# ziesha-network/bazuka

Hardware: NVIDIA B200
Metric: g1_msm_scalars_per_sec (higher is better)
Workload: dtype u32x12 Montgomery (Fp) / u32x8 (Fr) on the GPU; u64 limbs on the CPU

## Files before the change

### bazuka_b200/csrc/ec.cuh

```cuda
#pragma once
#include "ff.cuh"

#if defined(__CUDACC__)
#define BZK_HD_COLD __host__ __device__ __noinline__
#else
#define BZK_HD_COLD
#endif

namespace bzk {

struct Fp2 {
    Fp c0, c1;
    BZK_HD static Fp2 zero() { return Fp2{Fp::zero(), Fp::zero()}; }
    BZK_HD static Fp2 one() { return Fp2{Fp::one(), Fp::zero()}; }
    BZK_HD bool is_zero() const { return c0.is_zero() && c1.is_zero(); }
    BZK_HD bool operator==(const Fp2 &o) const { return c0 == o.c0 && c1 == o.c1; }
    BZK_HD bool operator!=(const Fp2 &o) const { return !(*this == o); }
    BZK_HD friend Fp2 operator+(const Fp2 &a, const Fp2 &b) { return Fp2{a.c0 + b.c0, a.c1 + b.c1}; }
    BZK_HD friend Fp2 operator-(const Fp2 &a, const Fp2 &b) { return Fp2{a.c0 - b.c0, a.c1 - b.c1}; }
    BZK_HD Fp2 neg() const { return Fp2{c0.neg(), c1.neg()}; }
    BZK_HD Fp2 dbl() const { return Fp2{c0.dbl(), c1.dbl()}; }
    BZK_HD friend Fp2 operator*(const Fp2 &a, const Fp2 &b) {
        Fp t0 = a.c0 * b.c0;
        Fp t1 = a.c1 * b.c1;
        Fp t2 = (a.c0 + a.c1) * (b.c0 + b.c1);
        return Fp2{t0 - t1, t2 - t0 - t1};
    }
    BZK_HD Fp2 sqr() const {
        Fp t = c0 * c1;
        return Fp2{(c0 + c1) * (c0 - c1), t.dbl()};
    }
    BZK_HD Fp2 inv() const {
        Fp n = (c0.sqr() + c1.sqr()).inv();
        return Fp2{c0 * n, (c1 * n).neg()};
    }
};

template <class F>
struct Affine {
    F x, y;
    BZK_HD bool is_inf() const { return x.is_zero() && y.is_zero(); }
    BZK_HD static Affine inf() { return Affine{F::zero(), F::zero()}; }
    BZK_HD Affine neg() const { return Affine{x, y.neg()}; }
};

template <class F>
struct Xyzz {
    F X, Y, ZZ, ZZZ;

    BZK_HD static Xyzz inf() { return Xyzz{F::zero(), F::zero(), F::zero(), F::zero()}; }
    BZK_HD bool is_inf() const { return ZZ.is_zero(); }
    BZK_HD static Xyzz from_affine(const Affine<F> &p) {
        if (p.is_inf()) return inf();
        return Xyzz{p.x, p.y, F::one(), F::one()};
    }
    BZK_HD Xyzz neg() const { return Xyzz{X, Y.neg(), ZZ, ZZZ}; }

    BZK_HD_COLD static Xyzz dbl_affine(const Affine<F> &p) {
        if (p.is_inf() || p.y.is_zero()) return inf();
        F U = p.y.dbl();
        F V = U.sqr();
        F W = U * V;
        F S = p.x * V;
        F M = p.x.sqr();
        M = M.dbl() + M;
        Xyzz r;
        r.X = M.sqr() - S.dbl();
        r.Y = M * (S - r.X) - W * p.y;
        r.ZZ = V;
        r.ZZZ = W;
        return r;
    }
    BZK_HD_COLD Xyzz dbl() const {
        if (is_inf() || Y.is_zero()) return inf();
        F U = Y.dbl();
        F V = U.sqr();
        F W = U * V;
        F S = X * V;
        F M = X.sqr();
        M = M.dbl() + M;
        Xyzz r;
        r.X = M.sqr() - S.dbl();
        r.Y = M * (S - r.X) - W * Y;
        r.ZZ = V * ZZ;
        r.ZZZ = W * ZZZ;
        return r;
    }
    BZK_HD void madd(const Affine<F> &p) {
        if (p.is_inf()) return;
        if (is_inf()) {
            X = p.x; Y = p.y; ZZ = F::one(); ZZZ = F::one();
            return;
        }
        F Pd = p.x * ZZ - X;
        F Rd = p.y * ZZZ - Y;
        if (Pd.is_zero()) {
            if (Rd.is_zero()) *this = dbl_affine(p);
            else *this = inf();
            return;
        }
        F PP = Pd.sqr();
        F PPP = Pd * PP;
        F Q = X * PP;
        F X3 = Rd.sqr() - PPP - Q.dbl();
        Y = Rd * (Q - X3) - Y * PPP;
        X = X3;
        ZZ = ZZ * PP;
        ZZZ = ZZZ * PPP;
    }
    BZK_HD_COLD void add(const Xyzz &o) {
        if (o.is_inf()) return;
        if (is_inf()) { *this = o; return; }
        F U1 = X * o.ZZ;
        F U2 = o.X * ZZ;
        F S1 = Y * o.ZZZ;
        F S2 = o.Y * ZZZ;
        F Pd = U2 - U1;
        F Rd = S2 - S1;
        if (Pd.is_zero()) {
            if (Rd.is_zero()) *this = dbl();
            else *this = inf();
            return;
        }
        F PP = Pd.sqr();
        F PPP = Pd * PP;
        F Q = U1 * PP;
        F X3 = Rd.sqr() - PPP - Q.dbl();
        Y = Rd * (Q - X3) - S1 * PPP;
        X = X3;
        ZZ = ZZ * o.ZZ * PP;
        ZZZ = ZZZ * o.ZZZ * PPP;
    }
    BZK_HD_COLD Affine<F> to_affine() const {
        if (is_inf()) return Affine<F>::inf();
        F i = (ZZ * ZZZ).inv();
        return Affine<F>{X * ZZZ * i, Y * ZZ * i};
    }
};

template <class F>
BZK_HD F pair_denominator(const Affine<F> &a, const Affine<F> &b) {
    if (a.is_inf() || b.is_inf()) return F::one();
    const F dx = b.x - a.x;
    if (!dx.is_zero()) return dx;
    if (a.y == b.y && !a.y.is_zero()) return a.y.dbl();
    return F::one();
}
template <class F>
BZK_HD Affine<F> pair_sum(const Affine<F> &a, const Affine<F> &b, const F &dinv) {
    if (a.is_inf()) return b;
    if (b.is_inf()) return a;
    F lam;
    if (a.x != b.x) {
        lam = (b.y - a.y) * dinv;
    } else {
        if (!(a.y == b.y) || a.y.is_zero()) return Affine<F>::inf();
        const F xx = a.x.sqr();
        lam = (xx.dbl() + xx) * dinv;
    }
    Affine<F> r;
    r.x = lam.sqr() - a.x - b.x;
    r.y = lam * (a.x - r.x) - a.y;
    return r;
}

typedef Affine<Fp> G1Affine;
typedef Affine<Fp2> G2Affine;
typedef Xyzz<Fp> G1Xyzz;
typedef Xyzz<Fp2> G2Xyzz;

template <class F>
BZK_HD Xyzz<F> scalar_mul(const Affine<F> &p, const uint32_t k[8]) {
    Xyzz<F> acc = Xyzz<F>::inf();
    for (int i = 255; i >= 0; i--) {
        acc = acc.dbl();
        if ((k[i >> 5] >> (i & 31)) & 1) acc.madd(p);
    }
    return acc;
}

}
```

### bazuka_b200/csrc/ff.cuh

```cuda
#pragma once
#include <stdint.h>
#include <string.h>

#if defined(__CUDACC__)
#define BZK_HD __host__ __device__ __forceinline__
#define BZK_D __device__ __forceinline__
#else
#define BZK_HD inline
#define BZK_D inline
#endif

#if defined(__CUDACC__)
#define BZK_HD_POW __host__ __device__ __noinline__
#else
#define BZK_HD_POW
#endif

namespace bzk {

struct CC {
    uint32_t c;
};

#if defined(__CUDA_ARCH__)
// ... 98 lines not shown
        return r;
    }
    BZK_HD friend Fe operator+(const Fe &a, const Fe &b) {
#if defined(__CUDA_ARCH__)
        return add_limbs32(a, b);
#else
        return add_host64(a, b);
#endif
    }
    BZK_HD friend Fe operator-(const Fe &a, const Fe &b) {
#if defined(__CUDA_ARCH__)
        return sub_limbs32(a, b);
#else
        return sub_host64(a, b);
#endif
    }
    struct HostConsts {
        uint64_t p[N / 2];
        uint64_t inv64;
    };
    static inline const HostConsts &host_consts() {
        static const HostConsts hc = [] {
            HostConsts c;
            for (int i = 0; i < N / 2; i++) c.p[i] = (uint64_t)P::p(2 * i) | ((uint64_t)P::p(2 * i + 1) << 32);
            uint64_t x = (uint64_t)(0u - P::inv());
            x *= 2 - c.p[0] * x;
            c.inv64 = (uint64_t)0 - x;
            return c;
        }();
        return hc;
    }
    static inline Fe add_host64(const Fe &a, const Fe &b) {
        constexpr int M = N / 2;
        uint64_t A[M], B[M], t[M], s[M];
        memcpy(A, a.l, sizeof A);
        memcpy(B, b.l, sizeof B);
        unsigned __int128 c = 0;
        for (int i = 0; i < M; i++) { c += (unsigned __int128)A[i] + B[i]; t[i] = (uint64_t)c; c >>= 64; }
        uint64_t borrow = 0;
        const uint64_t *Pm = host_consts().p;
        for (int i = 0; i < M; i++) {
            const uint64_t pm = Pm[i];
            const unsigned __int128 d = (unsigned __int128)t[i] - pm - borrow;
            s[i] = (uint64_t)d;
            borrow = (uint64_t)(d >> 64) & 1;
        }
        Fe r;
        memcpy(r.l, borrow ? t : s, sizeof t);
        return r;
    }
    static inline Fe sub_host64(const Fe &a, const Fe &b) {
        constexpr int M = N / 2;
        uint64_t A[M], B[M], t[M];
        memcpy(A, a.l, sizeof A);
        memcpy(B, b.l, sizeof B);
        uint64_t borrow = 0;
        for (int i = 0; i < M; i++) {
            const unsigned __int128 d = (unsigned __int128)A[i] - B[i] - borrow;
            t[i] = (uint64_t)d;
            borrow = (uint64_t)(d >> 64) & 1;
        }
        if (borrow) {
            unsigned __int128 c = 0;
            const uint64_t *Pm = host_consts().p;
            for (int i = 0; i < M; i++) {
                const uint64_t pm = Pm[i];
                c += (unsigned __int128)t[i] + pm;
                t[i] = (uint64_t)c;
                c >>= 64;
            }
        }
        Fe r;
        memcpy(r.l, t, sizeof t);
        return r;
    }
    BZK_HD static Fe add_limbs32(const Fe &a, const Fe &b) {
        Fe t;
        CC cc{0};
        t.l[0] = add_cc(a.l[0], b.l[0], cc);
#pragma unroll
        for (int i = 1; i < N; i++) t.l[i] = addc_cc(a.l[i], b.l[i], cc);
        return reduce_once(t);
    }
    BZK_HD static Fe sub_limbs32(const Fe &a, const Fe &b) {
        Fe t;
        CC cc{0};
        t.l[0] = sub_cc(a.l[0], b.l[0], cc);
#pragma unroll
        for (int i = 1; i < N; i++) t.l[i] = subc_cc(a.l[i], b.l[i], cc);
        uint32_t borrow = subc(0, 0, cc);
        CC c2{0};
        t.l[0] = add_cc(t.l[0], borrow & P::p(0), c2);
#pragma unroll
        for (int i = 1; i < N; i++) t.l[i] = addc_cc(t.l[i], borrow & P::p(i), c2);
        return t;
    }
    BZK_HD Fe neg() const { return zero() - *this; }
    BZK_HD Fe dbl() const { return *this + *this; }

    BZK_HD friend Fe operator*(const Fe &a, const Fe &b) {
#if defined(__CUDA_ARCH__) && defined(BZK_MUL_NOINLINE)
        return mul_call(a, b);
#elif defined(__CUDA_ARCH__)
        return mul_evenodd(a, b);
#else
        return mul_host64(a, b);
#endif
    }
#if defined(__CUDACC__)
    __device__ __noinline__ static Fe mul_call(Fe a, Fe b) { return mul_evenodd(a, b); }
#endif
    static inline Fe mul_host64(const Fe &a, const Fe &b) {
        constexpr int M = N / 2;
        uint64_t A[M], B[M], t[M + 2];
        memcpy(A, a.l, sizeof A);
        memcpy(B, b.l, sizeof B);
        const HostConsts &hc = host_consts();
        const uint64_t *Pm = hc.p;
        const uint64_t inv64 = hc.inv64;
        for (int i = 0; i < M + 2; i++) t[i] = 0;
        for (int i = 0; i < M; i++) {
            unsigned __int128 cur;
            uint64_t carry = 0;
            for (int j = 0; j < M; j++) {
                cur = (unsigned __int128)A[j] * B[i] + t[j] + carry;
                t[j] = (uint64_t)cur;
                carry = (uint64_t)(cur >> 64);
            }
            cur = (unsigned __int128)t[M] + carry;
            t[M] = (uint64_t)cur;
            t[M + 1] = (uint64_t)(cur >> 64);
            const uint64_t m = t[0] * inv64;
            cur = (unsigned __int128)m * Pm[0] + t[0];
            carry = (uint64_t)(cur >> 64);
            for (int j = 1; j < M; j++) {
                cur = (unsigned __int128)m * Pm[j] + t[j] + carry;
                t[j - 1] = (uint64_t)cur;
                carry = (uint64_t)(cur >> 64);
            }
            cur = (unsigned __int128)t[M] + carry;
            t[M - 1] = (uint64_t)cur;
            t[M] = t[M + 1] + (uint64_t)(cur >> 64);
        }
        uint64_t s[M], borrow = 0;
        for (int i = 0; i < M; i++) {
            const unsigned __int128 d = (unsigned __int128)t[i] - Pm[i] - borrow;
            s[i] = (uint64_t)d;
            borrow = (uint64_t)(d >> 64) & 1;
        }
        Fe r;
        memcpy(r.l, borrow ? t : s, M * sizeof(uint64_t));
        return r;
    }
    BZK_HD static Fe mul_evenodd(const Fe &a, const Fe &b) {
        uint32_t E[2 * N + 2], O[2 * N + 2];
#pragma unroll
        for (int i = 0; i < 2 * N + 2; i++) E[i] = O[i] = 0;
        CC cc{0};
#pragma unroll
        for (int i = 0; i < N; i++) {
            uint32_t *Pp = (i & 1) ? O : E;
            uint32_t *Q = (i & 1) ? E : O;
            const uint32_t bi = b.l[i];
            if (i == 0) {
#pragma unroll
                for (int j = 0; j < N; j += 2) {
                    Pp[j] = mul_lo(a.l[j], bi);
                    Pp[j + 1] = mul_hi(a.l[j], bi);
                    Q[j + 1] = mul_lo(a.l[j + 1], bi);
                    Q[j + 2] = mul_hi(a.l[j + 1], bi);
                }
            } else {
                Pp[i] = add_cc(Pp[i], Q[i], cc);
#pragma unroll
                for (int j = 1; j < N; j += 2) mad_pair_next(Q[i + j], Q[i + j + 1], a.l[j], bi, cc);
                Q[i + N + 1] = addc(0, 0, cc);
                mad_pair_first(Pp[i], Pp[i + 1], a.l[0], bi, cc);
#pragma unroll
                for (int j = 2; j < N; j += 2) mad_pair_next(Pp[i + j], Pp[i + j + 1], a.l[j], bi, cc);
                Pp[i + N] = addc(Pp[i + N], 0, cc);
            }
            const uint32_t m = mul_lo(Pp[i], P::inv());
            mad_pair_first(Pp[i], Pp[i + 1], m, P::p(0), cc);
#pragma unroll
            for (int j = 2; j < N; j += 2) mad_pair_next(Pp[i + j], Pp[i + j + 1], m, P::p(j), cc);
            Pp[i + N] = addc(Pp[i + N], 0, cc);
            mad_pair_first(Q[i + 1], Q[i + 2], m, P::p(1), cc);
#pragma unroll
            for (int j = 3; j < N; j += 2) mad_pair_next(Q[i + j], Q[i + j + 1], m, P::p(j), cc);
            Q[i + N + 1] = addc(Q[i + N + 1], 0, cc);
        }
        Fe r;
        r.l[0] = add_cc(E[N], O[N], cc);
#pragma unroll
        for (int k = 1; k < N; k++) r.l[k] = addc_cc(E[N + k], O[N + k], cc);
        return reduce_once(r);
    }
    BZK_HD Fe sqr() const { return (*this) * (*this); }

    BZK_HD static void mul_wide(uint32_t out[2 * N], const Fe &a, const Fe &b) {
        uint32_t E[2 * N + 2], O[2 * N + 2];
#pragma unroll
        for (int i = 0; i < 2 * N + 2; i++) E[i] = O[i] = 0;
        CC cc{0};
#pragma unroll
        for (int i = 0; i < N; i++) {
            uint32_t *Pp = (i & 1) ? O : E;
            uint32_t *Q = (i & 1) ? E : O;
            const uint32_t bi = b.l[i];
            if (i == 0) {
#pragma unroll
                for (int j = 0; j < N; j += 2) {
                    Pp[j] = mul_lo(a.l[j], bi);
                    Pp[j + 1] = mul_hi(a.l[j], bi);
                    Q[j + 1] = mul_lo(a.l[j + 1], bi);
                    Q[j + 2] = mul_hi(a.l[j + 1], bi);
                }
            } else {
                mad_pair_first(Q[i + 1], Q[i + 2], a.l[1], bi, cc);
#pragma unroll
                for (int j = 3; j < N; j += 2) mad_pair_next(Q[i + j], Q[i + j + 1], a.l[j], bi, cc);
                Q[i + N + 1] = addc(0, 0, cc);
                mad_pair_first(Pp[i], Pp[i + 1], a.l[0], bi, cc);
#pragma unroll
                for (int j = 2; j < N; j += 2) mad_pair_next(Pp[i + j], Pp[i + j + 1], a.l[j], bi, cc);
                Pp[i + N] = addc(Pp[i + N], 0, cc);
            }
        }
        out[0] = add_cc(E[0], O[0], cc);
#pragma unroll
        for (int k = 1; k < 2 * N; k++) out[k] = addc_cc(E[k], O[k], cc);
    }
    BZK_HD static void wide_accumulate(uint32_t acc[2 * N + 1], const uint32_t w[2 * N]) {
        CC cc{0};
        acc[0] = add_cc(acc[0], w[0], cc);
#pragma unroll
        for (int k = 1; k < 2 * N; k++) acc[k] = addc_cc(acc[k], w[k], cc);
        acc[2 * N] = addc(acc[2 * N], 0, cc);
    }
    BZK_HD static Fe redc_wide(const uint32_t T[2 * N + 1]) {
        uint32_t t[2 * N + 2];
#pragma unroll
        for (int k = 0; k < 2 * N + 1; k++) t[k] = T[k];
        t[2 * N + 1] = 0;
#pragma unroll
        for (int i = 0; i < N + 1; i++) {
            const uint32_t m = t[i] * P::inv();
            uint64_t carry = 0;
#pragma unroll
            for (int j = 0; j < N; j++) {
                uint64_t cur = (uint64_t)m * P::p(j) + t[i + j] + carry;
                t[i + j] = (uint32_t)cur;
                carry = cur >> 32;
            }
#pragma unroll
            for (int k = i + N; k < 2 * N + 2; k++) {
                uint64_t cur = (uint64_t)t[k] + carry;
                t[k] = (uint32_t)cur;
                carry = cur >> 32;
            }
        }
        Fe r;
#pragma unroll
        for (int k = 0; k < N; k++) r.l[k] = t[N + 1 + k];
        return reduce_once(r);
    }

    BZK_HD Fe to_mont() const { return (*this) * r2(); }
    BZK_HD Fe from_mont() const {
        Fe o = zero();
        o.l[0] = 1;
        return (*this) * o;
    }
    BZK_HD static Fe from_u32(uint32_t v) {
        Fe o = zero();
        o.l[0] = v;
        return o.to_mont();
    }
    BZK_HD_POW Fe pow(const uint32_t *e, int nw) const {
        Fe acc = one();
        for (int i = nw * 32 - 1; i >= 0; i--) {
            acc = acc.sqr();
            if ((e[i >> 5] >> (i & 31)) & 1) acc = acc * (*this);
        }
        return acc;
    }
    BZK_HD Fe inv() const {
        uint32_t e[N];
#pragma unroll
        for (int i = 0; i < N; i++) e[i] = P::p(i);
        uint32_t borrow = 2;
        for (int i = 0; i < N && borrow; i++) {
            uint32_t before = e[i];
            e[i] = before - borrow;
            borrow = before < borrow ? 1 : 0;
        }
        return pow(e, N);
    }
    BZK_HD_POW Fe inv_gcd() const {
        if (is_zero()) return zero();
        uint32_t u[N], v[N], x1[N], x2[N];
#pragma unroll
        for (int i = 0; i < N; i++) { u[i] = l[i]; v[i] = P::p(i); x1[i] = 0; x2[i] = 0; }
        x1[0] = 1;
        auto is_one = [](const uint32_t *a) {
            uint32_t t = a[0] ^ 1u;
#pragma unroll
            for (int i = 1; i < N; i++) t |= a[i];
            return t == 0;
        };
        auto halve = [](uint32_t *a, uint32_t *x) {
#pragma unroll
            for (int i = 0; i < N - 1; i++) a[i] = (a[i] >> 1) | (a[i + 1] << 31);
            a[N - 1] >>= 1;
            uint32_t top = 0;
            if (x[0] & 1u) {
                CC cc{0};
                x[0] = add_cc(x[0], P::p(0), cc);
#pragma unroll
                for (int i = 1; i < N; i++) x[i] = addc_cc(x[i], P::p(i), cc);
                top = addc(0, 0, cc);
            }
#pragma unroll
            for (int i = 0; i < N - 1; i++) x[i] = (x[i] >> 1) | (x[i + 1] << 31);
            x[N - 1] = (x[N - 1] >> 1) | (top << 31);
        };
        auto sub_mod = [](uint32_t *x, const uint32_t *y) {
            CC cc{0};
            x[0] = sub_cc(x[0], y[0], cc);
#pragma unroll
            for (int i = 1; i < N; i++) x[i] = subc_cc(x[i], y[i], cc);
            if (subc(0, 0, cc)) {
                CC c2{0};
                x[0] = add_cc(x[0], P::p(0), c2);
#pragma unroll
                for (int i = 1; i < N - 1; i++) x[i] = addc_cc(x[i], P::p(i), c2);
                x[N - 1] = addc(x[N - 1], P::p(N - 1), c2);
            }
        };
        while (!is_one(u) && !is_one(v)) {
            while (!(u[0] & 1u)) halve(u, x1);
            while (!(v[0] & 1u)) halve(v, x2);
            uint32_t d[N];
            CC cc{0};
            d[0] = sub_cc(u[0], v[0], cc);
#pragma unroll
            for (int i = 1; i < N; i++) d[i] = subc_cc(u[i], v[i], cc);
            if (!subc(0, 0, cc)) {
#pragma unroll
                for (int i = 0; i < N; i++) u[i] = d[i];
                sub_mod(x1, x2);
// ... 48 lines not shown
```

### bazuka_b200/csrc/msm_impl.cuh

```cuda
#pragma once
#include "common.cuh"
#include "msm_affine.cuh"
#include <cstdlib>
#ifndef BZK_ACC_MIN_BLOCKS_G1
#define BZK_ACC_MIN_BLOCKS_G1 4
#endif

namespace bzk {


constexpr double kReduceCost = 6.0, kNarrowTopCost = 1.5;
static double plan_cost(size_t n, uint32_t c, uint32_t T) {
    const uint32_t W = (256 + c - 1) / c;
    const uint32_t Te = T < W ? T : W, G = (W + Te - 1) / Te;
    const int top_bits = 255 - (int)(c * (W - 1));
    const double narrow = (W > 1 && top_bits < 10 && n >= 4096) ? kNarrowTopCost * (double)n : 0.0;
    return (double)n * W + kReduceCost * G * (double)(1u << (c - 1)) + narrow;
}
static MsmPlan make_plan(size_t n, uint32_t c_tab = 0, uint32_t T = 1, uint32_t G_tab = 0) {
    uint32_t best_c = c_tab;
    if (!c_tab) {
        double best = 1e300;
        for (uint32_t c = 2; c <= 18; c++) {
            double cost = plan_cost(n, c, 1);
// ... 22 lines not shown
        double cost = plan_cost(n, c, T);
        if (cost < best) { best = cost; bc = c; bT = T; }
    }
    const uint32_t W = (256 + bc - 1) / bc;
    *c_out = bc;
    *G_out = (W + bT - 1) / bT;
    *T_out = (W + *G_out - 1) / *G_out;
}

__host__ __device__ __forceinline__ int32_t signed_digit(const uint32_t k[8], uint32_t c, uint32_t w, uint32_t &carry) {
    const uint32_t pos = w * c;
    uint32_t raw = 0;
    if (pos < 256) {
        const uint32_t limb = pos >> 5, sh = pos & 31;
        uint64_t two = k[limb];
        if (limb + 1 < 8) two |= (uint64_t)k[limb + 1] << 32;
        raw = (uint32_t)(two >> sh) & ((1u << c) - 1);
    }
    raw += carry;
    if (raw > (1u << (c - 1))) {
        carry = 1;
        return (int32_t)raw - (int32_t)(1u << c);
    }
    carry = 0;
    return (int32_t)raw;
}

template <bool SCATTER>
__global__ void __launch_bounds__(256) k_digits(const Fr *__restrict__ scalars, size_t n, uint32_t c, uint32_t W, uint32_t NB, uint32_t G,
                                                uint32_t n_tab, uint32_t off, uint32_t *__restrict__ counts_or_cursor, uint32_t *__restrict__ sorted) {
    const size_t i = (size_t)blockIdx.x * blockDim.x + threadIdx.x;
    if (i >= n) return;
    Fr k = load_vec(scalars + i).from_mont();
    uint32_t carry = 0;
    for (uint32_t w = 0; w < W; w++) {
        int32_t d = signed_digit(k.l, c, w, carry);
        if (d == 0) continue;
        uint32_t neg = d < 0;
        uint32_t b = (uint32_t)(neg ? -d : d) - 1;
        const uint32_t t = w / G, g = w - t * G;
        uint32_t slot = g * NB + b;
        if (SCATTER) {
            uint32_t pos = atomicAdd(&counts_or_cursor[slot], 1u);
            sorted[pos] = (t * n_tab + off + (uint32_t)i) | (neg << 31);
        } else {
            atomicAdd(&counts_or_cursor[slot], 1u);
        }
    }
}

constexpr int kScanBlock = 256, kScanItems = 4, kScanTile = kScanBlock * kScanItems;

static __global__ void __launch_bounds__(kScanBlock) k_scan_tile_sums(const uint32_t *__restrict__ in, uint32_t count, uint32_t *__restrict__ tile_sums) {
    __shared__ uint32_t sh[kScanBlock / 32];
    uint32_t base = blockIdx.x * kScanTile + threadIdx.x * kScanItems;
    uint32_t s = 0;
#pragma unroll
    for (int k = 0; k < kScanItems; k++)
        if (base + k < count) s += in[base + k];
#pragma unroll
    for (int o = 16; o > 0; o >>= 1) s += __shfl_down_sync(0xffffffffu, s, o);
    if ((threadIdx.x & 31) == 0) sh[threadIdx.x >> 5] = s;
    __syncthreads();
    if (threadIdx.x == 0) {
        uint32_t t = 0;
        for (int k = 0; k < kScanBlock / 32; k++) t += sh[k];
        tile_sums[blockIdx.x] = t;
    }
}
static __global__ void __launch_bounds__(1024) k_scan_tiles(uint32_t *__restrict__ tile_sums, uint32_t ntiles) {
    __shared__ uint32_t sh[1024];
    __shared__ uint32_t carry;
    if (threadIdx.x == 0) carry = 0;
    __syncthreads();
    for (uint32_t base = 0; base < ntiles; base += 1024) {
        uint32_t idx = base + threadIdx.x;
        uint32_t v = idx < ntiles ? tile_sums[idx] : 0;
        sh[threadIdx.x] = v;
        __syncthreads();
        for (uint32_t o = 1; o < 1024; o <<= 1) {
            uint32_t t = threadIdx.x >= o ? sh[threadIdx.x - o] : 0;
            __syncthreads();
            sh[threadIdx.x] += t;
            __syncthreads();
        }
        uint32_t incl = sh[threadIdx.x];
        if (idx < ntiles) tile_sums[idx] = carry + incl - v;
        __syncthreads();
        if (threadIdx.x == 1023) carry += incl;
        __syncthreads();
    }
    if (threadIdx.x == 0) tile_sums[ntiles] = carry;
}
static __global__ void __launch_bounds__(kScanBlock) k_scan_apply(const uint32_t *__restrict__ in, uint32_t count, const uint32_t *__restrict__ tile_sums,
                                                           uint32_t ntiles, uint32_t *__restrict__ offsets, uint32_t *__restrict__ cursor) {
    __shared__ uint32_t sh[kScanBlock];
    uint32_t base = blockIdx.x * kScanTile + threadIdx.x * kScanItems;
    uint32_t v[kScanItems], s = 0;
#pragma unroll
    for (int k = 0; k < kScanItems; k++) { v[k] = (base + k < count) ? in[base + k] : 0; s += v[k]; }
    sh[threadIdx.x] = s;
    __syncthreads();
    for (uint32_t o = 1; o < kScanBlock; o <<= 1) {
        uint32_t t = threadIdx.x >= o ? sh[threadIdx.x - o] : 0;
        __syncthreads();
        sh[threadIdx.x] += t;
        __syncthreads();
    }
    uint32_t run = tile_sums[blockIdx.x] + sh[threadIdx.x] - s;
#pragma unroll
    for (int k = 0; k < kScanItems; k++) {
        if (base + k < count) { offsets[base + k] = run; cursor[base + k] = run; }
        run += v[k];
    }
    if (blockIdx.x == 0 && threadIdx.x == 0) offsets[count] = tile_sums[ntiles];
}

__device__ __forceinline__ uint32_t effective_chunk(uint32_t M, uint32_t threads, uint32_t min_chunk) {
    uint32_t c = (M + threads - 1) / threads;
    return c < min_chunk ? min_chunk : c;
}

template <class F> struct AccBlocks { static constexpr int value = 1; };
template <> struct AccBlocks<Fp> { static constexpr int value = BZK_ACC_MIN_BLOCKS_G1; };

template <class F>
__global__ void __launch_bounds__(128, AccBlocks<F>::value) k_accumulate(const Affine<F> *__restrict__ bases, const Affine<F> *__restrict__ scr, const uint32_t *__restrict__ sorted,
                                                    const uint32_t *__restrict__ offsets, uint32_t TB, uint32_t min_chunk,
                                                    Xyzz<F> *__restrict__ buckets, Xyzz<F> *__restrict__ part_pts,
                                                    int32_t *__restrict__ part_bucket) {
    const uint32_t t = blockIdx.x * blockDim.x + threadIdx.x;
    const uint32_t M = offsets[TB];
    const uint32_t chunk = effective_chunk(M, gridDim.x * blockDim.x, min_chunk);
    const uint64_t start64 = (uint64_t)t * chunk;
    part_bucket[2 * t] = -1;
    part_bucket[2 * t + 1] = -1;
    if (start64 >= M) return;
    const uint32_t start = (uint32_t)start64;
    const uint32_t end = (uint32_t)(start64 + chunk < M ? start64 + chunk : M);
    uint32_t lo = 0, hi = TB;
    while (hi - lo > 1) {
        uint32_t mid = (lo + hi) >> 1;
        if (offsets[mid] <= start) lo = mid; else hi = mid;
    }
    uint32_t b = lo;
    uint32_t bend = offsets[b + 1];
    while (bend <= start) { b++; bend = offsets[b + 1]; }
    uint32_t run_start = start;
    bool run_from_bucket_start = (offsets[b] == start);
    Xyzz<F> acc = Xyzz<F>::inf();
    for (uint32_t pos = start; pos < end; pos++) {
        if (pos == bend) {
            if (run_from_bucket_start) {
                store_vec(buckets + b, acc);
            } else {
                const uint32_t slot = 2 * t + (run_start == start ? 0 : 1);
                store_vec(part_pts + slot, acc);
                part_bucket[slot] = (int32_t)b;
            }
            acc = Xyzz<F>::inf();
            do { b++; bend = offsets[b + 1]; } while (bend <= pos);
            run_start = pos;
            run_from_bucket_start = true;
        }
        const uint32_t e = sorted[pos];
        Affine<F> p;
        if (scr) {
            p = load_ref(bases, scr, e);
        } else {
            p = load_vec(bases + (e & 0x7fffffffu));
            if (e >> 31) p.y = p.y.neg();
        }
        acc.madd(p);
    }
    if (run_from_bucket_start && bend == end) {
        store_vec(buckets + b, acc);
    } else {
        const uint32_t slot = 2 * t + (run_start == start ? 0 : 1);
        store_vec(part_pts + slot, acc);
        part_bucket[slot] = (int32_t)b;
    }
}

constexpr uint32_t kLongRun = 6;
constexpr uint32_t kLongQueueCap = 4096;
struct LongRun { uint32_t first, last; int32_t bucket; uint32_t pad; };

template <class F>
__global__ void __launch_bounds__(128) k_fixup(const Xyzz<F> *__restrict__ part_pts, const int32_t *__restrict__ part_bucket,
                                               uint32_t nslots_max, const uint32_t *__restrict__ offsets, uint32_t TB, uint32_t acc_threads, uint32_t min_chunk,
                                               Xyzz<F> *__restrict__ buckets,
                                               LongRun *__restrict__ queue, uint32_t *__restrict__ queue_len) {
    const uint32_t e = blockIdx.x * blockDim.x + threadIdx.x;
    const uint32_t M = offsets[TB];
    const uint32_t chunk = effective_chunk(M, acc_threads, min_chunk);
    uint32_t nslots = 2 * ((M + chunk - 1) / chunk);
    if (nslots > nslots_max) nslots = nslots_max;
    if (e >= nslots) return;
    const int32_t b = part_bucket[e];
    if (b < 0) return;
    for (uint32_t q = e; q-- > 0;) {
        int32_t pb = part_bucket[q];
        if (pb < 0) continue;
        if (pb == b) return;
        break;
    }
    uint32_t last = e, count = 1;
    for (uint32_t q = e + 1; q < nslots; q++) {
        int32_t nb = part_bucket[q];
        if (nb < 0) continue;
        if (nb != b) break;
        last = q;
        count++;
    }
    if (count > kLongRun) {
        uint32_t at = atomicAdd(queue_len, 1u);
        if (at < kLongQueueCap) {
            queue[at] = LongRun{e, last, b, 0};
            return;
        }
    }
    Xyzz<F> acc = load_vec(part_pts + e);
    for (uint32_t q = e + 1; q <= last; q++)
        if (part_bucket[q] == b) acc.add(load_vec(part_pts + q));
    store_vec(buckets + b, acc);
}

template <class F>
__global__ void __launch_bounds__(256) k_fixup_long(const Xyzz<F> *__restrict__ part_pts, const int32_t *__restrict__ part_bucket,
                                                    Xyzz<F> *__restrict__ buckets, const LongRun *__restrict__ queue,
                                                    const uint32_t *__restrict__ queue_len) {
    extern __shared__ uint4 smem_raw[];
    Xyzz<F> *sh = (Xyzz<F> *)smem_raw;
    uint32_t nq = *queue_len;
    if (nq > kLongQueueCap) nq = kLongQueueCap;
    for (uint32_t r = blockIdx.x; r < nq; r += gridDim.x) {
        const LongRun run = queue[r];
        Xyzz<F> acc = Xyzz<F>::inf();
        for (uint32_t q = run.first + threadIdx.x; q <= run.last; q += blockDim.x)
            if (part_bucket[q] == run.bucket) acc.add(load_vec(part_pts + q));
        sh[threadIdx.x] = acc;
        __syncthreads();
        for (uint32_t o = blockDim.x / 2; o > 0; o >>= 1) {
            if (threadIdx.x < o) {
                Xyzz<F> a = sh[threadIdx.x];
                a.add(sh[threadIdx.x + o]);
                sh[threadIdx.x] = a;
            }
            __syncthreads();
        }
        if (threadIdx.x == 0) store_vec(buckets + run.bucket, sh[0]);
        __syncthreads();
    }
}

template <class F>
__global__ void __launch_bounds__(128) k_bucket_slices(const Xyzz<F> *__restrict__ buckets, uint32_t NB, uint32_t slice, uint32_t nslices_total,
                                                       Xyzz<F> *__restrict__ acc_out, Xyzz<F> *__restrict__ run_out) {
    const uint32_t g = blockIdx.x * blockDim.x + threadIdx.x;
    if (g >= nslices_total) return;
    const uint32_t per_win = (NB + slice - 1) / slice;
    const uint32_t w = g / per_win, sidx = g % per_win;
    const uint32_t lo = sidx * slice;
    const uint32_t len = (lo + slice <= NB) ? slice : NB - lo;
    const Xyzz<F> *B = buckets + (size_t)w * NB;
    Xyzz<F> run = Xyzz<F>::inf(), acc = Xyzz<F>::inf();
    for (uint32_t k = len; k-- > 0;) {
        run.add(load_vec(B + lo + k));
        acc.add(run);
    }
    store_vec(acc_out + g, acc);
    store_vec(run_out + g, run);
}

constexpr uint32_t kCombineThreads = 64, kCombineSerial = 8, kCombineSpan = kCombineThreads * kCombineSerial;
template <class F>
__global__ void __launch_bounds__(kCombineThreads) k_slice_combine(const Xyzz<F> *__restrict__ acc_in, const Xyzz<F> *__restrict__ run_in, uint32_t per_win,
                                                                  Xyzz<F> *__restrict__ partial) {
    extern __shared__ uint4 smem_raw[];
    Xyzz<F> *sh = (Xyzz<F> *)smem_raw;
    const uint32_t j = blockIdx.y, g = blockIdx.z;
    Xyzz<F> v = Xyzz<F>::inf();
    for (uint32_t k = 0; k < kCombineSerial; k++) {
        const uint32_t s = blockIdx.x * kCombineSpan + k * kCombineThreads + threadIdx.x;
        if (s >= per_win) break;
        if (j == 0) v.add(load_vec(acc_in + (size_t)g * per_win + s));
        else if ((s >> (j - 1)) & 1) v.add(load_vec(run_in + (size_t)g * per_win + s));
    }
    sh[threadIdx.x] = v;
    __syncthreads();
    for (uint32_t o = kCombineThreads / 2; o > 0; o >>= 1) {
        if (threadIdx.x < o) {
            Xyzz<F> a = sh[threadIdx.x];
            a.add(sh[threadIdx.x + o]);
            sh[threadIdx.x] = a;
        }
        __syncthreads();
    }
    if (threadIdx.x == 0) store_vec(partial + ((size_t)(g * gridDim.y + j)) * gridDim.x + blockIdx.x, sh[0]);
}
template <class F>
__global__ void __launch_bounds__(128) k_partial_sum(const Xyzz<F> *__restrict__ partial, uint32_t parts, Xyzz<F> *__restrict__ win_out) {
    extern __shared__ uint4 smem_raw[];
    Xyzz<F> *sh = (Xyzz<F> *)smem_raw;
    const size_t row = blockIdx.x;
    Xyzz<F> acc = Xyzz<F>::inf();
    for (uint32_t k = threadIdx.x; k < parts; k += blockDim.x) acc.add(load_vec(partial + row * parts + k));
    sh[threadIdx.x] = acc;
    __syncthreads();
    for (uint32_t o = blockDim.x / 2; o > 0; o >>= 1) {
        if (threadIdx.x < o) {
            Xyzz<F> a = sh[threadIdx.x];
            a.add(sh[threadIdx.x + o]);
            sh[threadIdx.x] = a;
        }
        __syncthreads();
    }
    if (threadIdx.x == 0) store_vec(win_out + row, sh[0]);
}

static __global__ void __launch_bounds__(256) k_pack_g1(const uint8_t *__restrict__ images, size_t n, G1Affine *__restrict__ out, uint32_t *bad) {
    const size_t i = (size_t)blockIdx.x * blockDim.x + threadIdx.x;
    if (i >= n) return;
    G1Affine p = load_g1_image(images + i * 104);
    if (bad && !p.is_inf()) {
        Fp rhs = p.x.sqr() * p.x + Fp::from_u32(4);
        if (p.y.sqr() != rhs) atomicAdd(bad, 1u);
    }
    store_vec(out + i, p);
}
static __global__ void __launch_bounds__(128) k_pack_g2(const uint8_t *__restrict__ images, size_t n, G2Affine *__restrict__ out, uint32_t *bad) {
    const size_t i = (size_t)blockIdx.x * blockDim.x + threadIdx.x;
    if (i >= n) return;
    G2Affine p = load_g2_image(images + i * 200);
    if (bad && !p.is_inf()) {
        Fp four = Fp::from_u32(4);
        Fp2 rhs = p.x.sqr() * p.x + Fp2{four, four};
        if (p.y.sqr() != rhs) atomicAdd(bad, 1u);
    }
    store_vec(out + i, p);
}

static __global__ void __launch_bounds__(128) k_random_g1(uint64_t seed, size_t n, G1Affine gen, uint8_t *__restrict__ out) {
    const size_t i = (size_t)blockIdx.x * blockDim.x + threadIdx.x;
    if (i >= n) return;
    Fr k = splitmix_fr_canonical(seed, i);
    store_g1_image(out + i * 104, scalar_mul(gen, k.l).to_affine());
}
static __global__ void __launch_bounds__(64) k_random_g2(uint64_t seed, size_t n, G2Affine gen, uint8_t *__restrict__ out) {
    const size_t i = (size_t)blockIdx.x * blockDim.x + threadIdx.x;
    if (i >= n) return;
    Fr k = splitmix_fr_canonical(seed, i);
    store_g2_image(out + i * 200, scalar_mul(gen, k.l).to_affine());
}
static __global__ void __launch_bounds__(256) k_random_fr(uint64_t seed, size_t n, Fr *__restrict__ out) {
    const size_t i = (size_t)blockIdx.x * blockDim.x + threadIdx.x;
    if (i >= n) return;
    store_vec(out + i, splitmix_fr_canonical(seed, i).to_mont());
}

static Fp fp_from_hex(const char *hex96) {
    Fp v;
    for (int i = 0; i < 12; i++) {
        uint32_t x = 0;
        for (int k = 0; k < 8; k++) {
            char ch = hex96[(11 - i) * 8 + k];
            x = (x << 4) | (uint32_t)(ch <= '9' ? ch - '0' : (ch | 32) - 'a' + 10);
        }
        v.l[i] = x;
    }
    return v.to_mont();
}
static G1Affine g1_generator() {
    return G1Affine{
        fp_from_hex("17f1d3a73197d7942695638c4fa9ac0fc3688c4f9774b905a14e3a3f171bac586c55e83ff97a1aeffb3af00adb22c6bb"),
        fp_from_hex("08b3f481e3aaa0f1a09e30ed741d8ae4fcf5e095d5d00af600db18cb2c04b3edd03cc744a2888ae40caa232946c5e7e1")};
}
static G2Affine g2_generator() {
    return G2Affine{
        Fp2{fp_from_hex("024aa2b2f08f0a91260805272dc51051c6e47ad4fa403b02b4510b647ae3d1770bac0326a805bbefd48056c8c121bdb8"),
            fp_from_hex("13e02b6052719f607dacd3a088274f65596bd0d09920b61ab5da61bbdc7f5049334cf11213945d57e5ac7d055d042b7e")},
        Fp2{fp_from_hex("0ce5d527727d6e118cc9cdc6da2e351aadfd9baa8cbdd3a76d429a695160d12c923ac9cc3baca289e193548608b82801"),
            fp_from_hex("0606c4a02ea734cc32acd2b02bc28b99cb3e287e85a763af267492ab572e99ab3f370d275cec1da1aaa9075ff05f79be")}};
}

static G1Affine g1_from_image(const bzk_g1_affine *img) {
    if (img->infinity) return G1Affine::inf();
    G1Affine p;
    memcpy(p.x.l, img->x, 48);
    memcpy(p.y.l, img->y, 48);
    return p;
}
static void g1_to_image(bzk_g1_affine *img, const G1Affine &p) {
    memset(img, 0, sizeof *img);
    if (p.is_inf()) {
        Fp one = Fp::one();
        memcpy(img->y, one.l, 48);
        img->infinity = 1;
        return;
    }
    memcpy(img->x, p.x.l, 48);
    memcpy(img->y, p.y.l, 48);
}
static G2Affine g2_from_image(const bzk_g2_affine *img) {
    if (img->infinity) return G2Affine::inf();
    G2Affine p;
    memcpy(p.x.c0.l, img->x, 48);
    memcpy(p.x.c1.l, img->x + 6, 48);
    memcpy(p.y.c0.l, img->y, 48);
    memcpy(p.y.c1.l, img->y + 6, 48);
    return p;
}
static void g2_to_image(bzk_g2_affine *img, const G2Affine &p) {
    memset(img, 0, sizeof *img);
    if (p.is_inf()) {
        Fp one = Fp::one();
        memcpy(img->y, one.l, 48);
        img->infinity = 1;
        return;
    }
    memcpy(img->x, p.x.c0.l, 48);
    memcpy(img->x + 6, p.x.c1.l, 48);
    memcpy(img->y, p.y.c0.l, 48);
    memcpy(img->y + 6, p.y.c1.l, 48);
}
template <class F> struct Wire;
template <> struct Wire<Fp> {
    typedef bzk_g1_affine image;
    static void to_image(image *i, const Affine<Fp> &p) { g1_to_image(i, p); }
    static Affine<Fp> from_image(const image *i) { return g1_from_image(i); }
};
template <> struct Wire<Fp2> {
    typedef bzk_g2_affine image;
    static void to_image(image *i, const Affine<Fp2> &p) { g2_to_image(i, p); }
    static Affine<Fp2> from_image(const image *i) { return g2_from_image(i); }
};

constexpr uint32_t kMaxLevels = 16;
template <class F>
__global__ void __launch_bounds__(128) k_precompute(Affine<F> *__restrict__ tab, size_t n, uint32_t T, uint32_t bits) {
    const size_t i = (size_t)blockIdx.x * blockDim.x + threadIdx.x;
    if (i >= n) return;
    const Affine<F> P = load_vec(tab + i);
    Xyzz<F> L[kMaxLevels - 1];
    F pre[kMaxLevels - 1];
    Xyzz<F> acc = Xyzz<F>::from_affine(P);
    F run = F::one();
    for (uint32_t t = 1; t < T; t++) {
        for (uint32_t k = 0; k < bits; k++) acc = acc.dbl();
        L[t - 1] = acc;
        pre[t - 1] = run;
        if (!acc.is_inf()) run = run * (acc.ZZ * acc.ZZZ);
    }
    F inv = run.inv();
    for (uint32_t t = T - 1; t >= 1; t--) {
        const Xyzz<F> &Q = L[t - 1];
        Affine<F> out = Affine<F>::inf();
        if (!Q.is_inf()) {
            const F qi = inv * pre[t - 1];
            inv = inv * (Q.ZZ * Q.ZZZ);
            out.x = Q.X * Q.ZZZ * qi;
            out.y = Q.Y * Q.ZZ * qi;
        }
        store_vec(tab + (size_t)t * n + i, out);
    }
}

template <class F>
static int32_t bases_precompute(bzk_ctx *ctx, Affine<F> **d, size_t n, uint32_t max_levels, uint32_t *c_out, uint32_t *T_out, uint32_t *G_out) {
    if (max_levels > kMaxLevels) max_levels = kMaxLevels;
    uint32_t c = 0, T = 1, G = 0;
// ... 244 lines not shown
```

Before: 139.4 million.

## Use lazy-reduced field arithmetic in G1 bucket accumulation and reduction kernels

Introduces weak (redundant, < 2p) Montgomery arithmetic for Fp: mul without final conditional subtraction, add/sub/neg modulo 2p, a dedicated squaring that exploits symmetric cross products, and a fused two-product multiply-sum for the Y coordinate. Bucket accumulation, merge, and window reduction kernels switch to madd_weak/add_weak and canonicalise only when storing results. This is meant to remove per-operation final reductions and some multiply work from the hot point-addition loops. The risk is correctness in zero checks and bound tracking, since values can hold representations up to 2p and the doubling path relies on canonicalisation.

```diff
diff --git a/bazuka_b200/csrc/ec.cuh b/bazuka_b200/csrc/ec.cuh
--- a/bazuka_b200/csrc/ec.cuh
+++ b/bazuka_b200/csrc/ec.cuh
@@ -1,4 +1,5 @@
 #pragma once
+#include <type_traits>
 #include "ff.cuh"
 
 #if defined(__CUDACC__)
@@ -131,6 +132,63 @@
         ZZ = ZZ * o.ZZ * PP;
         ZZZ = ZZZ * o.ZZZ * PPP;
     }
+
+    BZK_HD Xyzz canon() const {
+        if constexpr (std::is_same<F, Fp>::value) return Xyzz{F::canon(X), F::canon(Y), F::canon(ZZ), F::canon(ZZZ)};
+        else return *this;
+    }
+    BZK_HD void madd_weak(const Affine<F> &p) {
+        if constexpr (!std::is_same<F, Fp>::value) {
+            madd(p);
+        } else {
+            if (p.is_inf()) return;
+            if (ZZ.is_zero_weak()) {
+                X = p.x; Y = p.y; ZZ = F::one(); ZZZ = F::one();
+                return;
+            }
+            const F Pd = F::sub_weak(F::mul_weak(p.x, ZZ), X);
+            const F Rd = F::sub_weak(F::mul_weak(p.y, ZZZ), Y);
+            if (Pd.is_zero_weak()) {
+                if (Rd.is_zero_weak()) *this = dbl_affine(p);
+                else *this = inf();
+                return;
+            }
+            const F PP = F::sqr_weak(Pd);
+            const F PPP = F::mul_weak(Pd, PP);
+            const F Q = F::mul_weak(X, PP);
+            ZZ = F::mul_weak(ZZ, PP);
+            X = F::sub_weak(F::sub_weak(F::sqr_weak(Rd), PPP), F::add_weak(Q, Q));
+            Y = F::mul2_sum_weak(Rd, F::sub_weak(Q, X), F::neg_weak(Y), PPP);
+            ZZZ = F::mul_weak(ZZZ, PPP);
+        }
+    }
+    BZK_HD_COLD void add_weak(const Xyzz &o) {
+        if constexpr (!std::is_same<F, Fp>::value) {
+            add(o);
+        } else {
+            if (o.ZZ.is_zero_weak()) return;
+            if (ZZ.is_zero_weak()) { *this = o; return; }
+            const F U1 = F::mul_weak(X, o.ZZ);
+            const F U2 = F::mul_weak(o.X, ZZ);
+            const F S1 = F::mul_weak(Y, o.ZZZ);
+            const F S2 = F::mul_weak(o.Y, ZZZ);
+            const F Pd = F::sub_weak(U2, U1);
+            const F Rd = F::sub_weak(S2, S1);
+            if (Pd.is_zero_weak()) {
+                if (Rd.is_zero_weak()) *this = canon().dbl();
+                else *this = inf();
+                return;
+            }
+            const F PP = F::sqr_weak(Pd);
+            const F PPP = F::mul_weak(Pd, PP);
+            const F Q = F::mul_weak(U1, PP);
+            const F X3 = F::sub_weak(F::sub_weak(F::sqr_weak(Rd), PPP), F::add_weak(Q, Q));
+            Y = F::mul2_sum_weak(Rd, F::sub_weak(Q, X3), F::neg_weak(S1), PPP);
+            X = X3;
+            ZZ = F::mul_weak(F::mul_weak(ZZ, o.ZZ), PP);
+            ZZZ = F::mul_weak(F::mul_weak(ZZZ, o.ZZZ), PPP);
+        }
+    }
     BZK_HD_COLD Affine<F> to_affine() const {
         if (is_inf()) return Affine<F>::inf();
         F i = (ZZ * ZZZ).inv();
diff --git a/bazuka_b200/csrc/ff.cuh b/bazuka_b200/csrc/ff.cuh
--- a/bazuka_b200/csrc/ff.cuh
+++ b/bazuka_b200/csrc/ff.cuh
@@ -274,7 +274,59 @@
         memcpy(r.l, borrow ? t : s, M * sizeof(uint64_t));
         return r;
     }
-    BZK_HD static Fe mul_evenodd(const Fe &a, const Fe &b) {
+    BZK_HD static Fe mul_evenodd(const Fe &a, const Fe &b) { return reduce_once(mul_weak(a, b)); }
+
+    BZK_HD static constexpr uint32_t p2(int i) {
+        return (P::p(i) << 1) | (i ? P::p(i - 1) >> 31 : 0u);
+    }
+    BZK_HD static Fe canon(const Fe &a) { return reduce_once(a); }
+    BZK_HD bool is_zero_weak() const {
+        uint32_t z = 0, q = 0;
+#pragma unroll
+        for (int i = 0; i < N; i++) { z |= l[i]; q |= l[i] ^ P::p(i); }
+        return z == 0 || q == 0;
+    }
+    BZK_HD static Fe add_weak(const Fe &a, const Fe &b) {
+        Fe s, t;
+        CC cc{0};
+        s.l[0] = add_cc(a.l[0], b.l[0], cc);
+#pragma unroll
+        for (int i = 1; i < N; i++) s.l[i] = addc_cc(a.l[i], b.l[i], cc);
+        CC c2{0};
+        t.l[0] = sub_cc(s.l[0], p2(0), c2);
+#pragma unroll
+        for (int i = 1; i < N; i++) t.l[i] = subc_cc(s.l[i], p2(i), c2);
+        const uint32_t borrow = subc(0, 0, c2);
+#pragma unroll
+        for (int i = 0; i < N; i++) t.l[i] = borrow ? s.l[i] : t.l[i];
+        return t;
+    }
+    BZK_HD static Fe sub_weak(const Fe &a, const Fe &b) {
+        Fe t;
+        CC cc{0};
+        t.l[0] = sub_cc(a.l[0], b.l[0], cc);
+#pragma unroll
+        for (int i = 1; i < N; i++) t.l[i] = subc_cc(a.l[i], b.l[i], cc);
+        const uint32_t borrow = subc(0, 0, cc);
+        CC c2{0};
+        t.l[0] = add_cc(t.l[0], borrow & p2(0), c2);
+#pragma unroll
+        for (int i = 1; i < N; i++) t.l[i] = addc_cc(t.l[i], borrow & p2(i), c2);
+        return t;
+    }
+    BZK_HD static Fe neg_weak(const Fe &a) {
+        Fe t;
+        CC cc{0};
+        t.l[0] = sub_cc(p2(0), a.l[0], cc);
+#pragma unroll
+        for (int i = 1; i < N; i++) t.l[i] = subc_cc(p2(i), a.l[i], cc);
+        return t;
+    }
+    BZK_HD static Fe mul_weak(const Fe &a, const Fe &b) { return mont_rows<false>(a, b, a, b); }
+    BZK_HD static Fe mul2_sum_weak(const Fe &a, const Fe &b, const Fe &c, const Fe &d) { return mont_rows<true>(a, b, c, d); }
+
+    template <bool TWO>
+    BZK_HD static Fe mont_rows(const Fe &a, const Fe &b, const Fe &c, const Fe &d) {
         uint32_t E[2 * N + 2], O[2 * N + 2];
 #pragma unroll
         for (int i = 0; i < 2 * N + 2; i++) E[i] = O[i] = 0;
@@ -302,6 +354,17 @@
                 for (int j = 2; j < N; j += 2) mad_pair_next(Pp[i + j], Pp[i + j + 1], a.l[j], bi, cc);
                 Pp[i + N] = addc(Pp[i + N], 0, cc);
             }
+            if (TWO) {
+                const uint32_t di = d.l[i];
+                mad_pair_first(Q[i + 1], Q[i + 2], c.l[1], di, cc);
+#pragma unroll
+                for (int j = 3; j < N; j += 2) mad_pair_next(Q[i + j], Q[i + j + 1], c.l[j], di, cc);
+                Q[i + N + 1] = addc(Q[i + N + 1], 0, cc);
+                mad_pair_first(Pp[i], Pp[i + 1], c.l[0], di, cc);
+#pragma unroll
+                for (int j = 2; j < N; j += 2) mad_pair_next(Pp[i + j], Pp[i + j + 1], c.l[j], di, cc);
+                Pp[i + N] = addc(Pp[i + N], 0, cc);
+            }
             const uint32_t m = mul_lo(Pp[i], P::inv());
             mad_pair_first(Pp[i], Pp[i + 1], m, P::p(0), cc);
 #pragma unroll
@@ -316,9 +379,69 @@
         r.l[0] = add_cc(E[N], O[N], cc);
 #pragma unroll
         for (int k = 1; k < N; k++) r.l[k] = addc_cc(E[N + k], O[N + k], cc);
-        return reduce_once(r);
+        return r;
     }
     BZK_HD Fe sqr() const { return (*this) * (*this); }
+
+    BZK_HD static Fe sqr_weak(const Fe &a) {
+        uint32_t E[2 * N + 2], O[2 * N + 2];
+#pragma unroll
+        for (int i = 0; i < 2 * N + 2; i++) E[i] = O[i] = 0;
+        CC cc{0};
+#pragma unroll
+        for (int i = 0; i < N - 1; i++) {
+            const uint32_t ai = a.l[i];
+            {
+                int top = i + 1;
+                mad_pair_first(O[2 * i + 1], O[2 * i + 2], a.l[i + 1], ai, cc);
+#pragma unroll
+                for (int j = i + 3; j < N; j += 2) { mad_pair_next(O[i + j], O[i + j + 1], a.l[j], ai, cc); top = j; }
+                O[i + top + 2] = addc(O[i + top + 2], 0, cc);
+            }
+            if (i + 2 < N) {
+                int top = i + 2;
+                mad_pair_first(E[2 * i + 2], E[2 * i + 3], a.l[i + 2], ai, cc);
+#pragma unroll
+                for (int j = i + 4; j < N; j += 2) { mad_pair_next(E[i + j], E[i + j + 1], a.l[j], ai, cc); top = j; }
+                E[i + top + 2] = addc(E[i + top + 2], 0, cc);
+            }
+        }
+        uint32_t T[2 * N];
+        T[0] = add_cc(E[0], O[0], cc);
+#pragma unroll
+        for (int k = 1; k < 2 * N; k++) T[k] = addc_cc(E[k], O[k], cc);
+#pragma unroll
+        for (int k = 2 * N - 1; k > 0; k--) T[k] = (T[k] << 1) | (T[k - 1] >> 31);
+        T[0] <<= 1;
+        mad_pair_first(T[0], T[1], a.l[0], a.l[0], cc);
+#pragma unroll
+        for (int i = 1; i < N; i++) mad_pair_next(T[2 * i], T[2 * i + 1], a.l[i], a.l[i], cc);
+#pragma unroll
+        for (int k = 0; k < 2 * N + 2; k++) { E[k] = k < N ? T[k] : 0u; O[k] = 0; }
+#pragma unroll
+        for (int i = 0; i < N; i++) {
+            uint32_t *Pp = (i & 1) ? O : E;
+            uint32_t *Q = (i & 1) ? E : O;
+            const uint32_t m = mul_lo(Pp[i] + Q[i], P::inv());
+            Pp[i] = add_cc(Pp[i], Q[i], cc);
+#pragma unroll
+            for (int j = 1; j < N; j += 2) mad_pair_next(Q[i + j], Q[i + j + 1], m, P::p(j), cc);
+            Q[i + N + 1] = addc(Q[i + N + 1], 0, cc);
+            mad_pair_first(Pp[i], Pp[i + 1], m, P::p(0), cc);
+#pragma unroll
+            for (int j = 2; j < N; j += 2) mad_pair_next(Pp[i + j], Pp[i + j + 1], m, P::p(j), cc);
+            Pp[i + N] = addc(Pp[i + N], 0, cc);
+        }
+        Fe r;
+        r.l[0] = add_cc(E[N], O[N], cc);
+#pragma unroll
+        for (int k = 1; k < N; k++) r.l[k] = addc_cc(E[N + k], O[N + k], cc);
+        CC c2{0};
+        r.l[0] = add_cc(r.l[0], T[N], c2);
+#pragma unroll
+        for (int k = 1; k < N; k++) r.l[k] = addc_cc(r.l[k], T[N + k], c2);
+        return r;
+    }
 
     BZK_HD static void mul_wide(uint32_t out[2 * N], const Fe &a, const Fe &b) {
         uint32_t E[2 * N + 2], O[2 * N + 2];
diff --git a/bazuka_b200/csrc/msm_impl.cuh b/bazuka_b200/csrc/msm_impl.cuh
--- a/bazuka_b200/csrc/msm_impl.cuh
+++ b/bazuka_b200/csrc/msm_impl.cuh
@@ -198,10 +198,10 @@
     for (uint32_t pos = start; pos < end; pos++) {
         if (pos == bend) {
             if (run_from_bucket_start) {
-                store_vec(buckets + b, acc);
+                store_vec(buckets + b, acc.canon());
             } else {
                 const uint32_t slot = 2 * t + (run_start == start ? 0 : 1);
-                store_vec(part_pts + slot, acc);
+                store_vec(part_pts + slot, acc.canon());
                 part_bucket[slot] = (int32_t)b;
             }
             acc = Xyzz<F>::inf();
@@ -217,13 +217,13 @@
             p = load_vec(bases + (e & 0x7fffffffu));
             if (e >> 31) p.y = p.y.neg();
         }
-        acc.madd(p);
+        acc.madd_weak(p);
     }
     if (run_from_bucket_start && bend == end) {
-        store_vec(buckets + b, acc);
+        store_vec(buckets + b, acc.canon());
     } else {
         const uint32_t slot = 2 * t + (run_start == start ? 0 : 1);
-        store_vec(part_pts + slot, acc);
+        store_vec(part_pts + slot, acc.canon());
         part_bucket[slot] = (int32_t)b;
     }
 }
@@ -268,8 +268,8 @@
     }
     Xyzz<F> acc = load_vec(part_pts + e);
     for (uint32_t q = e + 1; q <= last; q++)
-        if (part_bucket[q] == b) acc.add(load_vec(part_pts + q));
-    store_vec(buckets + b, acc);
+        if (part_bucket[q] == b) acc.add_weak(load_vec(part_pts + q));
+    store_vec(buckets + b, acc.canon());
 }
 
 template <class F>
@@ -284,18 +284,18 @@
         const LongRun run = queue[r];
         Xyzz<F> acc = Xyzz<F>::inf();
         for (uint32_t q = run.first + threadIdx.x; q <= run.last; q += blockDim.x)
-            if (part_bucket[q] == run.bucket) acc.add(load_vec(part_pts + q));
+            if (part_bucket[q] == run.bucket) acc.add_weak(load_vec(part_pts + q));
         sh[threadIdx.x] = acc;
         __syncthreads();
         for (uint32_t o = blockDim.x / 2; o > 0; o >>= 1) {
             if (threadIdx.x < o) {
                 Xyzz<F> a = sh[threadIdx.x];
-                a.add(sh[threadIdx.x + o]);
+                a.add_weak(sh[threadIdx.x + o]);
                 sh[threadIdx.x] = a;
             }
             __syncthreads();
         }
-        if (threadIdx.x == 0) store_vec(buckets + run.bucket, sh[0]);
+        if (threadIdx.x == 0) store_vec(buckets + run.bucket, sh[0].canon());
         __syncthreads();
     }
 }
@@ -312,11 +312,11 @@
     const Xyzz<F> *B = buckets + (size_t)w * NB;
     Xyzz<F> run = Xyzz<F>::inf(), acc = Xyzz<F>::inf();
     for (uint32_t k = len; k-- > 0;) {
-        run.add(load_vec(B + lo + k));
-        acc.add(run);
-    }
-    store_vec(acc_out + g, acc);
-    store_vec(run_out + g, run);
+        run.add_weak(load_vec(B + lo + k));
+        acc.add_weak(run);
+    }
+    store_vec(acc_out + g, acc.canon());
+    store_vec(run_out + g, run.canon());
 }
 
 constexpr uint32_t kCombineThreads = 64, kCombineSerial = 8, kCombineSpan = kCombineThreads * kCombineSerial;
@@ -330,20 +330,20 @@
     for (uint32_t k = 0; k < kCombineSerial; k++) {
         const uint32_t s = blockIdx.x * kCombineSpan + k * kCombineThreads + threadIdx.x;
         if (s >= per_win) break;
-        if (j == 0) v.add(load_vec(acc_in + (size_t)g * per_win + s));
-        else if ((s >> (j - 1)) & 1) v.add(load_vec(run_in + (size_t)g * per_win + s));
+        if (j == 0) v.add_weak(load_vec(acc_in + (size_t)g * per_win + s));
+        else if ((s >> (j - 1)) & 1) v.add_weak(load_vec(run_in + (size_t)g * per_win + s));
     }
     sh[threadIdx.x] = v;
     __syncthreads();
     for (uint32_t o = kCombineThreads / 2; o > 0; o >>= 1) {
         if (threadIdx.x < o) {
             Xyzz<F> a = sh[threadIdx.x];
-            a.add(sh[threadIdx.x + o]);
+            a.add_weak(sh[threadIdx.x + o]);
             sh[threadIdx.x] = a;
         }
         __syncthreads();
     }
-    if (threadIdx.x == 0) store_vec(partial + ((size_t)(g * gridDim.y + j)) * gridDim.x + blockIdx.x, sh[0]);
+    if (threadIdx.x == 0) store_vec(partial + ((size_t)(g * gridDim.y + j)) * gridDim.x + blockIdx.x, sh[0].canon());
 }
 template <class F>
 __global__ void __launch_bounds__(128) k_partial_sum(const Xyzz<F> *__restrict__ partial, uint32_t parts, Xyzz<F> *__restrict__ win_out) {
@@ -351,18 +351,18 @@
     Xyzz<F> *sh = (Xyzz<F> *)smem_raw;
     const size_t row = blockIdx.x;
     Xyzz<F> acc = Xyzz<F>::inf();
-    for (uint32_t k = threadIdx.x; k < parts; k += blockDim.x) acc.add(load_vec(partial + row * parts + k));
+    for (uint32_t k = threadIdx.x; k < parts; k += blockDim.x) acc.add_weak(load_vec(partial + row * parts + k));
     sh[threadIdx.x] = acc;
     __syncthreads();
     for (uint32_t o = blockDim.x / 2; o > 0; o >>= 1) {
         if (threadIdx.x < o) {
             Xyzz<F> a = sh[threadIdx.x];
-            a.add(sh[threadIdx.x + o]);
+            a.add_weak(sh[threadIdx.x + o]);
             sh[threadIdx.x] = a;
         }
         __syncthreads();
     }
-    if (threadIdx.x == 0) store_vec(win_out + row, sh[0]);
+    if (threadIdx.x == 0) store_vec(win_out + row, sh[0].canon());
 }
 
 static __global__ void __launch_bounds__(256) k_pack_g1(const uint8_t *__restrict__ images, size_t n, G1Affine *__restrict__ out, uint32_t *bad) {
```

New measurement: 147.1 million, median of 6. 5.6% higher.
